# natashabatalha/picaso

Measured on AMD Instinct MI355X. Metric: spectra/sec (1e5 wave x 90 layer reflected), higher is better.
Workload: dtype f64; 1 GPU; BASELINE configs[2]: Toon two-stream reflected light (get_reflected_1d + compress_disco), TTHG_ray, N=2, delta-Eddington, Rayleigh + cloud slab; nwno=100000, nlayer=90, gauss_angles=5, collective=none

## Files before the change

picaso_amd/csrc/api.hip:

```cpp
#include "common.hpp"
#include "planeseal.hpp"

#include <algorithm>
#include <cmath>
#include <cstdlib>

namespace pz {

thread_local char g_err[512] = {0};

int fail(picaso_ctx *ctx, const char *fmt, ...)
{
    char buf[512];
    va_list ap;
    va_start(ap, fmt);
    vsnprintf(buf, sizeof(buf), fmt, ap);
    va_end(ap);
    if (ctx) snprintf(ctx->err, sizeof(ctx->err), "%s", buf);
    snprintf(g_err, sizeof(g_err), "%s", buf);
    return 1;
}

int arena_reset(picaso_ctx *ctx, size_t need)
{
// ... 491 lines not shown
    g.iu0 = 1.0 / v0;
    g.iu0sq = 1.0 / (v0 * v0);
    g.nl0 = NL2E / v0; g.nl1 = NL2E / v1;
    g.nlm = NL2E * (1.0 / v0 + 1.0 / v1);
    g.wq2 = 2.0 * (v0 / (v0 + v1));
    g.q2 = (3.0 * 0.767 * 0.767 * v1 * v1 - 1.0) / 2.0;
    g.wgt = gw;
    g.wgt2 = tw;
    return g;
}

static double refl_dt_small(const double *ubar0, const double *ubar1, int count)
{
    if (getenv("PICASO_AMD_REFL_NO_SMALL_EXP") || !ubar0 || !ubar1 || count < 1) return -1.0;
    double umin = 1.0;
    for (int k = 0; k < count; ++k) {
        const double v0 = fabs(ubar0[k]), v1 = fabs(ubar1[k]);
        if (!(v0 > 0.0) || !(v1 > 0.0)) return -1.0;
        umin = fmin(umin, fmin(v0, v1));
    }
    return 0.34 * umin;
}

struct ReflBatchHost {
    int nspec;
    const double *const *plane[11];
    const double *const *surf_reflect, *const *F0PI;
    double *const *xint, *const *albedo;
    int ngeom;
    const double *cos_theta;
};

static bool reflected_seal_applies(picaso_ctx *ctx, int nlevel, int nwno, long plane_pitch, int numg, int numt,
                                   const double *const one[11], const double *ubar0, const double *ubar1, double cos_theta,
                                   int single_phase, int multi_phase, double frac_c, int toon_coefficients,
                                   const ReflBatchHost *bt, std::vector<unsigned long long> &masks, bool &use_masks)
{
    use_masks = false;
    const int nang = numg * numt, nspec = bt ? bt->nspec : 1, ngeom = bt ? bt->ngeom : 1;
    if (nang != 5) return false;
    for (int s = 0; s < ngeom; ++s) {
        const double ct = bt ? bt->cos_theta[s] : cos_theta;
        const double *u0 = ubar0 + (size_t)s * nang, *u1 = ubar1 + (size_t)s * nang;
        if (ct != 1.0) return false;
        for (int k = 0; k < nang; ++k)
            if (u0[k] != u1[k]) return false;
        if (!picaso_reflected_1d_can_derive(nlevel, plane_pitch, numg, numt, u0, u1, ct, single_phase, multi_phase, frac_c,
                                            toon_coefficients, 0))
            return false;
    }
    long coop_cols = 64L * ctx->ncu;
    if (const char *e = getenv("PICASO_AMD_REFL_COOP_COLS")) coop_cols = atol(e);
    const bool coop = !bt && nwno <= coop_cols && !getenv("PICASO_AMD_REFL_NO_COOP");
    if (!coop) {
        const int group = reflected_angle_group(ctx, nwno, nang, nspec);
        if (group == 1 || (group > 1 && group < nang && ((nang + group - 1) / group) * group <= MAX_ANGLES)) return false;
        if (angle_chunks(nang).size() != 1) return false;
        if ((long)nspec * ((nwno + 255L) / 256) * 4 <= 1024 && !getenv("PICASO_AMD_REFL_NO_BIG")) return false;
    }
    masks.assign(2 * (size_t)nspec, 0ull);
    bool all_valid = true, any_clear = false;
    for (int s = 0; s < nspec; ++s) {
        const double *pl[11];
        for (int j = 0; j < 11; ++j) pl[j] = bt ? bt->plane[j][s] : one[j];
        bool valid = false;
        if (!seal_derivable(ctx->device, pl, nlevel, nwno, plane_pitch, &masks[2 * (size_t)s], &valid)) return false;
        all_valid = all_valid && valid;
        any_clear = any_clear || masks[2 * (size_t)s] || masks[2 * (size_t)s + 1];
    }
    use_masks = !coop && all_valid && any_clear && !getenv("PICASO_AMD_REFL_NO_LAYER_MASK");
    return true;
}

static int reflected_1d_core(picaso_ctx *ctx, int nlevel, int nwno, int ncolper, long plane_pitch, int numg,
                                int numt, const double *dtau, const double *tau, const double *w0,
                                const double *cosb, const double *gcos2, const double *ftau_cld,
                                const double *ftau_ray, const double *dtau_og,
                                const double *tau_og, const double *w0_og, const double *cosb_og,
                                const double *surf_reflect, const double *ubar0,
                                const double *ubar1, double cos_theta, const double *F0PI,
                                int single_phase, int multi_phase, double frac_a, double frac_b,
                                double frac_c, double constant_back, double constant_forward,
                                int get_toa_intensity, int get_lvl_flux, int toon_coefficients,
                                double b_top, double *xint_at_top, double *flux_minus_all,
                                double *flux_plus_all, double *flux_minus_midpt_all,
                                double *flux_plus_midpt_all, const double *gweight,
                                const double *tweight, double *albedo, const ReflBatchHost *bt = nullptr)
{
    if (!ctx) return fail(nullptr, "null context");
    if (nlevel < 2 || nwno < 1 || numg < 1 || numt < 1)
        return fail(ctx, "get_reflected_1d: bad sizes nlevel=%d nwno=%d numg=%d numt=%d", nlevel, nwno, numg, numt);
    if (!dtau || !w0) return fail(ctx, "get_reflected_1d: dtau and w0 are required");
    if (!bt) PZ_NEED(ctx, "get_reflected_1d", surf_reflect, ubar0, ubar1, F0PI, xint_at_top);
    const bool clear_set = !ftau_cld;
    if (clear_set ? (cosb || cosb_og || ftau_ray || gcos2) : (!cosb || !cosb_og || !ftau_ray))
        return fail(ctx, "get_reflected_1d: cosb, cosb_og, ftau_cld, ftau_ray are given together or all left out (gcos2 "
                         "too in the second case)");
    if ((dtau_og == nullptr) != (w0_og == nullptr))
        return fail(ctx, "get_reflected_1d: dtau_og and w0_og are given together or both left out");
    const bool derived = !tau || !tau_og || !gcos2 || !ftau_cld || !dtau_og;
    if (derived && (get_lvl_flux || !get_toa_intensity))
        return fail(ctx, "get_reflected_1d: level fluxes need all eleven planes");
    const int nspec = bt ? bt->nspec : 1;
    const long ncol = (long)nwno * ncolper;
    if (plane_pitch < ncol) return fail(ctx, "get_reflected_1d: plane_pitch %ld < %ld columns", plane_pitch, ncol);
    if (ncolper > 1 && albedo)
        return fail(ctx, "get_reflected_1d: the fused disk sum is a per-wavelength output (ngauss = 1)");
    PZ_TRY(check_phase_options(ctx, single_phase, multi_phase, toon_coefficients));
    PZ_HIP(ctx, hipSetDevice(ctx->device));
    const int nang = numg * numt;
    ReflBatchHost bt_sealed;
    std::vector<const double *> absent;
    std::vector<unsigned long long> lmasks;
    bool use_lmask = false;
    if (!derived && ncolper == 1 && get_toa_intensity && !get_lvl_flux) {
        const double *const pl[11] = {dtau, tau, w0, cosb, gcos2, ftau_cld, ftau_ray, dtau_og, tau_og, w0_og, cosb_og};
        if (reflected_seal_applies(ctx, nlevel, nwno, plane_pitch, numg, numt, pl, ubar0, ubar1, cos_theta, single_phase,
                                   multi_phase, frac_c, toon_coefficients, bt, lmasks, use_lmask)) {
            tau = tau_og = gcos2 = nullptr;
            if (bt) {
                absent.assign((size_t)nspec, nullptr);
                bt_sealed = *bt;
                bt_sealed.plane[1] = bt_sealed.plane[4] = bt_sealed.plane[8] = absent.data();
                bt = &bt_sealed;
            }
            seal_count_hit(ctx->device, use_lmask);
        }
    }
    if (get_lvl_flux) {
        if (!flux_minus_all || !flux_plus_all || !flux_minus_midpt_all || !flux_plus_midpt_all)
            return fail(ctx, "get_reflected_1d: get_lvl_flux=1 needs the four level-flux outputs");
    }
    if (!get_toa_intensity) {
        PZ_HIP(ctx, hipMemsetAsync(xint_at_top, 0, sizeof(double) * (size_t)nang * ncol, ctx->stream));
        if (albedo) PZ_HIP(ctx, hipMemsetAsync(albedo, 0, sizeof(double) * nwno, ctx->stream));
        if (!get_lvl_flux) return 0;
    }
    ReflectedArgs a{};
    a.nlayer = nlevel - 1;
    a.ncol = ncol;
    a.ncolper = ncolper;
    a.pitch = plane_pitch;
    a.nfac = 1;
    a.nwno = nwno;
    a.dtau = dtau; a.tau = tau; a.w0 = w0; a.cosb = cosb; a.gcos2 = gcos2; a.ftau_cld = ftau_cld;
    a.ftau_ray = ftau_ray; a.dtau_og = dtau_og; a.tau_og = tau_og; a.w0_og = w0_og; a.cosb_og = cosb_og;
    a.surf_reflect = surf_reflect; a.F0PI = F0PI; a.cos_theta = cos_theta;
    a.single_phase = single_phase; a.multi_phase = multi_phase; a.toon_coefficients = toon_coefficients;
    a.frac_a = frac_a; a.frac_b = frac_b; a.frac_c = frac_c; a.constant_back = constant_back;
    a.constant_forward = constant_forward; a.b_top = b_top;
    a.use_lmask = use_lmask ? 1 : 0;
    if (use_lmask) { a.lmask[0] = lmasks[0]; a.lmask[1] = lmasks[1]; }
    a.dt_small = refl_dt_small(ubar0, ubar1, (bt ? bt->ngeom : 1) * nang);
    const bool fuse = albedo && gweight && tweight;
    a.albedo = fuse ? albedo : nullptr;
    a.albedo_scale = ((numt == 1) ? 2.0 * 3.14159265358979323846 : 1.0) * 0.5;
    std::vector<ReflBatchItem> items;
    auto upload_batch = [&](int first, int count, bool weights) -> int {
        items.resize((size_t)nspec);
        bool zp = true, ct1 = true;
        for (int s = 0; s < nspec; ++s) {
            ReflBatchItem &it = items[(size_t)s];
            const double *const *P[11];
            for (int j = 0; j < 11; ++j) P[j] = bt->plane[j];
            it.dtau = P[0][s]; it.tau = P[1][s]; it.w0 = P[2][s]; it.cosb = P[3][s]; it.gcos2 = P[4][s];
            it.ftau_cld = P[5][s]; it.ftau_ray = P[6][s]; it.dtau_og = P[7][s]; it.tau_og = P[8][s];
            it.w0_og = P[9][s]; it.cosb_og = P[10][s];
            it.surf_reflect = bt->surf_reflect[s]; it.F0PI = bt->F0PI[s];
            it.xint = bt->xint[s] + (size_t)first * ncol;
            it.albedo = (fuse && weights) ? bt->albedo[s] : nullptr;
            it.cos_theta = bt->cos_theta[bt->ngeom > 1 ? s : 0];
            it.u0_tab = it.u1_tab = nullptr;
            it.lmask[0] = use_lmask ? lmasks[2 * (size_t)s] : 0ull;
            it.lmask[1] = use_lmask ? lmasks[2 * (size_t)s + 1] : 0ull;
            ct1 = ct1 && it.cos_theta == 1.0;
            const double *u0 = ubar0 + (bt->ngeom > 1 ? (size_t)s * nang : 0), *u1 = ubar1 + (bt->ngeom > 1 ? (size_t)s * nang : 0);
            for (int k = 0; k < count; ++k) {
                const int idx = first + k < nang ? first + k : nang - 1;
                it.ang[k] = make_refl_angle(u0[idx], u1[idx], weights ? gweight[idx / numt] : 0.0,
                                            weights ? tweight[idx % numt] : 0.0);
                zp = zp && u0[idx] == u1[idx];
            }
        }
        const void *d = nullptr;
        PZ_TRY(table_upload(ctx, items.data(), sizeof(ReflBatchItem) * items.size(), &d));
        a.batch = (const ReflBatchItem *)d;
        a.nspec = nspec;
        a.batch_zp = zp ? 1 : 0;
        a.cos_theta = ct1 ? 1.0 : bt->cos_theta[0] == 1.0 ? 2.0 : bt->cos_theta[0];
        bool shared = nspec > 1;
        for (int s = 1; s < nspec && shared; ++s)
            for (int j = 0; j < 11; ++j) shared = shared && bt->plane[j][s] == bt->plane[j][0];
        a.batch_interleave = shared ? 1 : 0;
        return 0;
    };
    if (bt) {
        if (get_lvl_flux || !get_toa_intensity)
// ... 1019 lines not shown
```

picaso_amd/csrc/common.hpp:

```cpp
#pragma once
#include <hip/hip_runtime.h>

#include <initializer_list>

#include <unordered_map>

#include <cstdarg>
#include <cstdio>
#include <cstring>
#include <vector>

#include "../../include/picaso_hip.h"

namespace pz { struct PairwisePlan; }

struct picaso_ctx {
    int device = 0;
    hipStream_t stream = nullptr;
    hipEvent_t ev0 = nullptr, ev1 = nullptr;
    hipEvent_t wait_ev = nullptr;
    char err[512] = {0};
    int ncu = 256;
    char *arena = nullptr;
    size_t arena_bytes = 0, arena_used = 0;
// ... 83 lines not shown
constexpr int MAX_CK_GAUSS = 32;

struct ReflectedArgs {
    int nlayer;
    long ncol;
    int ncolper;
    long pitch;
    int nfac;
    int nwno;
    const double *dtau, *tau, *w0, *cosb, *gcos2, *ftau_cld, *ftau_ray, *dtau_og, *tau_og, *w0_og,
        *cosb_og;
    const double *surf_reflect, *F0PI;
    double cos_theta;
    int single_phase, multi_phase, toon_coefficients;
    double frac_a, frac_b, frac_c, constant_back, constant_forward, b_top;
    int na;
    int ny;
    int nvalid;
    int ncg;
    struct Angle {
        double u1, iu0, iu0sq, nl1, q2;
        double u0, nl0, nlm, wq2, wgt, wgt2;
    } ang[MAX_ANGLES];
    const double *u0_tab, *u1_tab;
    double *xint;
    double *albedo;
    double albedo_scale;
    int albedo_first, albedo_last;
    const struct ReflBatchItem *batch;
    int nspec;
    unsigned bps;
    int batch_zp;
    int batch_interleave;
    unsigned long long lmask[2];
    int use_lmask;
    double dt_small;
};
struct ReflBatchItem {
    const double *dtau, *tau, *w0, *cosb, *gcos2, *ftau_cld, *ftau_ray, *dtau_og, *tau_og, *w0_og, *cosb_og;
    const double *surf_reflect, *F0PI;
    double *xint, *albedo;
    double cos_theta;
    const double *u0_tab, *u1_tab;
    ReflectedArgs::Angle ang[MAX_ANGLES];
    unsigned long long lmask[2];
};
int launch_reflected_toa(picaso_ctx *ctx, const ReflectedArgs &a, bool is3d);
bool reflected_coop_ok(const ReflectedArgs &a);
int reflected_coop_pattern(const ReflectedArgs &a);
int launch_reflected_coop(picaso_ctx *ctx, const ReflectedArgs &a);
int launch_weighted_colsum(picaso_ctx *ctx, int nrows, long nwno, int n, const double *wts_host,
                           const double *in, double *out);
int launch_axpby(picaso_ctx *ctx, size_t n, double a, const double *x, double b, const double *y, double *out);


struct ThermalArgs {
    int nlayer;
    long ncol, pitch;
    int nfac, nwno;
    int ncolper;
    const double *wno, *dwno;
    const double *tlevel, *plevel;
    const double *dtau, *w0, *cosb;
    const double *surf_reflect;
    int hard_surface, calc_type;
    int na, ny;
// ... 50 lines not shown
```

picaso_amd/csrc/planeseal.hip:

```cpp
#include "common.hpp"
#include "planeseal.hpp"
#include "planeseal_registry.hpp"

namespace pz {

namespace {

using sealreg::Seal;
static_assert(sealreg::LEVELS_FLAGS == PICASO_SEAL_LEVELS, "planeseal_registry.hpp restates PICASO_SEAL_LEVELS");

sealreg::Registry &registry()
{
    static sealreg::Registry *r = new sealreg::Registry();
    return *r;
}

}

bool seal_derivable(int device, const double *const planes[11], int nlevel, int nwno, long pitch,
                    unsigned long long *layer_mask, bool *mask_valid)
{
    uint64_t m[2];
    const bool ok = registry().derivable(device, planes, nlevel, nwno, pitch, m, mask_valid);
    if (layer_mask) {
        layer_mask[0] = m[0];
        layer_mask[1] = m[1];
    }
    return ok;
}

void seal_count_hit(int device, bool with_layer_mask) { registry().count_hit(device, with_layer_mask); }

void seal_invalidate(int device, const void *p, size_t bytes) { registry().invalidate(device, p, bytes); }

void seal_drop_device(int device) { registry().drop_device(device); }

constexpr int SEAL_BLOCK = 256, SEAL_ROWS = 8;
static_assert(32 % SEAL_ROWS == 0, "the layers of one block lie inside one word of the mask");
constexpr int SEAL_WORDS = 1 + sealreg::MASK_LAYERS / 32;

__global__ __launch_bounds__(SEAL_BLOCK) void k_planes_seal(int nlayer, int nwno, long pitch, const double *dtau,
                                                             const double *tau, const double *gcos2,
                                                             const double *ftau_ray, const double *dtau_og,
                                                             const double *tau_og, const double *w0,
                                                             const double *ftau_cld, const double *w0_og, int *bad_out,
                                                             unsigned *notclear_out)
{
#pragma clang fp contract(off)
    const long col = (long)blockIdx.x * SEAL_BLOCK + threadIdx.x;
    if (col >= nwno) return;
    const int i0 = (int)blockIdx.y * SEAL_ROWS, i1 = (i0 + SEAL_ROWS < nlayer) ? i0 + SEAL_ROWS : nlayer;
    int bad = 0;
    unsigned notclear = 0;
    unsigned lane_cloudy = 0;
    double t = tau[(long)i0 * pitch + col], to = tau_og[(long)i0 * pitch + col];
    if (i0 == 0) {
        if (__double_as_longlong(t) != 0) bad |= PICASO_SEAL_TAU;
        if (__double_as_longlong(to) != 0) bad |= PICASO_SEAL_TAU_OG;
    }
#pragma unroll 4
    for (int i = i0; i < i1; ++i) {
        const long o = (long)i * pitch + col;
        const double tn = tau[o + pitch];
        const double dt = dtau[o], dto = dtau_og[o], fr = ftau_ray[o];
        if (!(tn == t + dt)) bad |= PICASO_SEAL_TAU;
        t = tn;
        if (i + 1 < nlayer) {
            const double ton = tau_og[o + pitch];
            if (!(ton == to + dto)) bad |= PICASO_SEAL_TAU_OG;
            to = ton;
        }
        if (!(gcos2[o] == 0.5 * fr)) bad |= PICASO_SEAL_GCOS2;
        if (notclear_out) {
            const bool cloudy = !(ftau_cld[o] == 0.0) || !(dto == dt) ||
                                __double_as_longlong(fr) != __double_as_longlong(1.0) ||
                                __double_as_longlong(w0_og[o]) != __double_as_longlong(w0[o]);
            if (cloudy) lane_cloudy |= 1u << (i - i0);
        }
    }
#pragma unroll
    for (int b = 0; b < SEAL_ROWS; ++b)
        if (__any((lane_cloudy >> b) & 1u)) notclear |= 1u << ((i0 & 31) + b);
    if (bad) atomicOr(bad_out, bad);
    if (notclear && (threadIdx.x & 63) == 0) atomicOr(notclear_out + (i0 >> 5), notclear);
}

}

using namespace pz;

extern "C" {

int picaso_reflected_planes_seal_dev(picaso_ctx *ctx, int nlevel, int nwno, long plane_pitch, const double *dtau,
                                     const double *tau, const double *w0, const double *cosb, const double *gcos2,
                                     const double *ftau_cld, const double *ftau_ray, const double *dtau_og,
                                     const double *tau_og, const double *w0_og, const double *cosb_og, int *flags_out)
{
    if (!ctx) return fail(nullptr, "null context");
    if (flags_out) *flags_out = 0;
    if (nlevel < 2 || nwno < 1) return fail(ctx, "reflected_planes_seal: bad sizes nlevel=%d nwno=%d", nlevel, nwno);
    if (plane_pitch < nwno) return fail(ctx, "reflected_planes_seal: plane_pitch %ld < %d columns", plane_pitch, nwno);
    PZ_NEED(ctx, "reflected_planes_seal", dtau, tau, w0, cosb, gcos2, ftau_cld, ftau_ray, dtau_og, tau_og, w0_og, cosb_og);
    PZ_HIP(ctx, hipSetDevice(ctx->device));
    void *word = nullptr;
    PZ_TRY(picaso_dev_malloc(ctx, sizeof(int) * SEAL_WORDS, &word));
    int found[SEAL_WORDS] = {0};
    const int nlayer = nlevel - 1;
    const bool with_mask = nlayer <= sealreg::MASK_LAYERS;
    auto run = [&]() -> int {
        PZ_HIP(ctx, hipMemsetAsync(word, 0, sizeof(int) * SEAL_WORDS, ctx->stream));
        const dim3 grid((unsigned)((nwno + SEAL_BLOCK - 1) / SEAL_BLOCK), (unsigned)((nlayer + SEAL_ROWS - 1) / SEAL_ROWS));
        hipLaunchKernelGGL(k_planes_seal, grid, dim3(SEAL_BLOCK), 0, ctx->stream, nlayer, nwno, plane_pitch, dtau, tau,
                           gcos2, ftau_ray, dtau_og, tau_og, w0, ftau_cld, w0_og, (int *)word,
                           with_mask ? (unsigned *)word + 1 : nullptr);
        PZ_HIP(ctx, hipGetLastError());
        PZ_HIP(ctx, hipMemcpyAsync(found, word, sizeof(int) * SEAL_WORDS, hipMemcpyDeviceToHost, ctx->stream));
        PZ_HIP(ctx, hipStreamSynchronize(ctx->stream));
        return 0;
    };
    const int rc = run();
    PZ_TRY(picaso_dev_free(ctx, word));
    if (rc) return rc;
    Seal s{};
    const double *pl[11] = {dtau, tau, w0, cosb, gcos2, ftau_cld, ftau_ray, dtau_og, tau_og, w0_og, cosb_og};
    for (int j = 0; j < 11; ++j) s.plane[j] = pl[j];
    s.nlevel = nlevel;
    s.nwno = nwno;
    s.pitch = plane_pitch;
    s.flags = PICASO_SEAL_LEVELS & ~found[0];
    sealreg::mask_from_device_words(s, with_mask ? (const unsigned *)found + 1 : nullptr);
    registry().record(ctx->device, s);
    if (flags_out) *flags_out = s.flags;
    return 0;
}

int picaso_reflected_planes_unseal(picaso_ctx *ctx, const void *any_plane_ptr)
{
    if (!ctx) return fail(nullptr, "null context");
    seal_invalidate(ctx->device, any_plane_ptr, 1);
    return 0;
}

int picaso_reflected_seal_stat(picaso_ctx *ctx, long *seals, long *hits)
{
    if (!ctx) return fail(nullptr, "null context");
    registry().stat(ctx->device, seals, hits, nullptr);
    return 0;
}

int picaso_reflected_seal_layers(picaso_ctx *ctx, const void *any_plane_ptr, int cap, int *clear_out, int *nlayer_out)
{
    if (!ctx) return fail(nullptr, "null context");
    if (!nlayer_out || cap < 0 || (cap > 0 && !clear_out)) return fail(ctx, "reflected_seal_layers: bad arguments");
// ... 13 lines not shown
```

picaso_amd/csrc/planeseal.hpp:

```cpp
#pragma once
#include <cstddef>

namespace pz {

bool seal_derivable(int device, const double *const planes[11], int nlevel, int nwno, long pitch,
                    unsigned long long *layer_mask = nullptr, bool *mask_valid = nullptr);
void seal_count_hit(int device, bool with_layer_mask = false);
void seal_invalidate(int device, const void *p, size_t bytes);
void seal_drop_device(int device);

}
```

picaso_amd/csrc/planeseal_registry.hpp:

```cpp
#pragma once
#include <atomic>
#include <cstddef>
#include <cstdint>
#include <map>
#include <mutex>
#include <vector>

namespace pz {
namespace sealreg {

constexpr int LEVELS_FLAGS = 7;
constexpr int MASK_LAYERS = 128;

struct Seal {
    const double *plane[11];
    int nlevel, nwno;
    long pitch;
    int flags;
    uint64_t clear[2];
    bool mask_valid;

    size_t extent(int j) const
    {
        const long rows = (j == 1 || j == 8) ? nlevel : nlevel - 1;
        return sizeof(double) * (size_t)((rows - 1) * pitch + nwno);
    }
    bool overlaps(const void *p, size_t bytes) const
    {
        const uintptr_t lo = (uintptr_t)p, hi = lo + bytes;
        for (int j = 0; j < 11; ++j) {
            const uintptr_t q = (uintptr_t)plane[j];
            if (lo < q + extent(j) && q < hi) return true;
        }
        return false;
    }
    bool same_set(const double *const p[11]) const
    {
        for (int j = 0; j < 11; ++j)
            if (plane[j] != p[j]) return false;
        return true;
    }
    bool sealed() const { return (flags & LEVELS_FLAGS) == LEVELS_FLAGS; }
    bool layer_clear(int i) const { return mask_valid && i >= 0 && i < MASK_LAYERS && ((clear[i >> 6] >> (i & 63)) & 1u); }
};

inline void mask_from_device_words(Seal &s, const unsigned *notclear)
{
    const int nlayer = s.nlevel - 1;
    s.clear[0] = s.clear[1] = 0;
    s.mask_valid = notclear != nullptr && nlayer <= MASK_LAYERS;
    if (!s.mask_valid) return;
    for (int i = 0; i < nlayer; ++i)
        if (!((notclear[i >> 5] >> (i & 31)) & 1u)) s.clear[i >> 6] |= (uint64_t)1 << (i & 63);
}

struct DeviceSeals {
    std::vector<Seal> seals;
    long hits = 0;
    long mask_launches = 0;
};

struct Registry {
    std::mutex mu;
    std::map<int, DeviceSeals> dev;
    std::atomic<long> records{0};

    long drop_where(DeviceSeals &d, bool (*pred)(const Seal &, const void *, size_t), const void *p, size_t bytes)
    {
        long n = 0;
        for (size_t k = d.seals.size(); k-- > 0;)
            if (pred(d.seals[k], p, bytes)) {
                d.seals.erase(d.seals.begin() + (long)k);
                ++n;
            }
        records -= n;
        return n;
    }

    void record(int device, const Seal &s)
    {
        std::lock_guard<std::mutex> lock(mu);
        DeviceSeals &d = dev[device];
        drop_where(d, [](const Seal &x, const void *q, size_t) { return x.same_set((const double *const *)q); }, s.plane, 0);
        d.seals.push_back(s);
        ++records;
    }

    bool derivable(int device, const double *const planes[11], int nlevel, int nwno, long pitch, uint64_t *mask,
                   bool *mask_valid)
    {
        if (mask) mask[0] = mask[1] = 0;
        if (mask_valid) *mask_valid = false;
        if (records.load(std::memory_order_relaxed) == 0) return false;
        std::lock_guard<std::mutex> lock(mu);
        auto it = dev.find(device);
        if (it == dev.end()) return false;
        for (const Seal &s : it->second.seals)
            if (s.same_set(planes)) {
                const bool ok = s.nlevel == nlevel && s.nwno == nwno && s.pitch == pitch && s.sealed();
                if (ok && s.mask_valid) {
                    if (mask) {
                        mask[0] = s.clear[0];
                        mask[1] = s.clear[1];
                    }
                    if (mask_valid) *mask_valid = true;
                }
                return ok;
            }
        return false;
    }

    void count_hit(int device, bool with_mask)
    {
        std::lock_guard<std::mutex> lock(mu);
        DeviceSeals &d = dev[device];
        ++d.hits;
        if (with_mask) ++d.mask_launches;
    }

    void invalidate(int device, const void *p, size_t bytes)
    {
        if (!p || !bytes || records.load(std::memory_order_relaxed) == 0) return;
        std::lock_guard<std::mutex> lock(mu);
        auto it = dev.find(device);
        if (it == dev.end()) return;
        drop_where(it->second, [](const Seal &s, const void *q, size_t n) { return s.overlaps(q, n); }, p, bytes);
    }

// ... 41 lines not shown
```

picaso_amd/csrc/toon_reflected.hip:

```cpp
#include "common.hpp"
#include "device_math.hpp"

namespace pz {

#ifndef PZ_REFL_MINWAVES
#define PZ_REFL_MINWAVES 2
#endif
#ifndef PZ_REFL_BLOCK
#define PZ_REFL_BLOCK 256
#endif

constexpr int NSTATE = 7;
enum { S_T = 0, S_XU, S_EO, S_KAPPA, S_ZETA, S_D1, S_D2 };
constexpr int LDS_MIN_ANGLES = 4;

#ifndef PZ_REFL_NLDS
#define PZ_REFL_NLDS 4
#endif

template <int NA, bool LDS>
struct ReflState {
    static constexpr int NL = LDS ? PZ_REFL_NLDS : 0;
    static constexpr int NR = NSTATE - NL;
    double reg[NR > 0 ? NR : 1][NA];
    double *lds;
    double rho, pgam, pEM;
    __device__ __forceinline__ double get(int var, int k) const
    {
        return (var >= NR) ? lds[((var - NR) * NA + k) * PZ_REFL_BLOCK] : reg[var < NR ? var : 0][k];
    }
    __device__ __forceinline__ void set(int var, int k, double v)
    {
        if (var >= NR) lds[((var - NR) * NA + k) * PZ_REFL_BLOCK] = v;
        else reg[var < NR ? var : 0][k] = v;
    }
};

struct LayerIn {
    double dt, tau_n, w0, g, gcos2, fc, fr, dto, tauo, w0o, cbo;
    bool cum_tau;
    bool eo_ok;
    bool same_dt;
    bool nocld;
    bool allf;
    bool af_cloud;
};

enum Body { BODY_GENERAL, BODY_CLOUD, BODY_CLEAR, BODY_CLEAR_TOP, BODY_CLEAR_TOP_SMALL };

template <int NA, bool IS3D, bool ZP, bool FIRST, bool LAST, bool LDS, bool FAST = false, Body KIND = BODY_GENERAL,
          bool XT = false>
__device__ __forceinline__ void reflected_layer(const ReflectedArgs &a, const LayerIn &L,
                                                ReflState<NA, LDS> &S,
                                                const ReflectedArgs::Angle (&g)[NA],
                                                const Exp2Coef &K, double F, double clip, int tc_,
                                                double b_top)
{
#pragma clang fp contract(off)
    constexpr bool NC = KIND >= BODY_CLEAR, AF = KIND != BODY_GENERAL, EOX = KIND >= BODY_CLEAR_TOP;
    constexpr bool SX = KIND == BODY_CLEAR_TOP_SMALL;
    constexpr int SDT = KIND == BODY_CLOUD ? 2 : 1;
    static_assert(!(XT || EOX) || (FAST && ZP), "XT, BODY_CLEAR_TOP*: the zero-phase default-options kernels only");
    const int tc = FAST ? 0 : tc_;
    const int single_phase = FAST ? 3 : a.single_phase;
    const int multi_phase = FAST ? 0 : a.multi_phase;
    const double cos_theta = (FAST && ZP) ? 1.0 : a.cos_theta;
    const double frac_c = FAST ? 2.0 : a.frac_c;
    const double dt = L.dt, w0 = L.w0;
    const double fcg = NC ? 0.0 : L.fc * L.g;
    double g1, g2, lam, lam2;
    if (NC) toon_gammas_nocld(tc, w0, g1, g2, lam, lam2);
    else toon_gammas(tc, w0, fcg, g1, g2, lam, lam2);
    const double E = fmin(lam * dt, clip);
    const double EP = fexp2(E * -NEG_LOG2E, K);
    const double r_ge = frcp(g2 * EP);
    const double ig2 = r_ge * EP, EM = r_ge * g2;
    const double gam = (g1 - lam) * ig2;
    double ps;
    if ((NC || L.nocld) && single_phase == 3)
        ps = L.fr * (0.75 * fma(cos_theta, cos_theta, 1.0));
    else
        ps = p_single<IS3D>(single_phase, L.cbo, L.gcos2, L.fc, L.fr, cos_theta, a.frac_a, a.frac_b,
                            frac_c, a.constant_back, a.constant_forward);
    const double ssa_h = (L.w0o * F * (0.125 / PI)) * ps;
    const double w2pi = w0 * (0.5 / PI);
    const double Fw0h = (0.5 * F) * w0;
    const double gcq = (multi_phase == 0) ? L.gcos2 : 0.0;
    const double c2 = NC ? 0.0 : ((tc == 1) ? 1.5 * fcg : SQ3 * fcg);
    const double A0 = NC ? (g1 + g2) : (g1 + g2) + c2;
    const double A1 = NC ? 0.0 : c2 * (g1 - g2);
    const double c15 = NC ? 0.0 : 1.5 * fcg;
    const double gp = 1.0 + gam;
    const double gmc = NC ? 0.0 : (1.0 - gam) * c15;
    const double w2gp = w2pi * gp, w2gmc = NC ? 0.0 : w2pi * gmc;
    const double w2A0 = w2pi * A0;

    double a1i = 0.0, a2i = 0.0, ia = 0.0, rho_n = gam, sfac = 0.0;
// ... 169 lines not shown
    const double F = a.F0PI[w], rs = a.surf_reflect[w];

    const double *p_dtau = a.dtau + col, *p_tau = a.tau + col, *p_w0 = a.w0 + col,
                 *p_cosb = a.cosb + col, *p_gcos2 = a.gcos2 + col, *p_fc = a.ftau_cld + col,
                 *p_fr = a.ftau_ray + col, *p_dto = a.dtau_og + col, *p_tauo = a.tau_og + col,
                 *p_w0o = a.w0_og + col, *p_cbo = a.cosb_og + col;

    constexpr bool LDS = (NA >= LDS_MIN_ANGLES) && !IS3D && !BIG;
    __shared__ double lds_state[LDS ? (PZ_REFL_NLDS > 0 ? PZ_REFL_NLDS : 1) * NA * PZ_REFL_BLOCK : 1];
    ReflState<NA, LDS> S;
    S.lds = lds_state + threadIdx.x;
    S.rho = S.pgam = S.pEM = 0.0;
    constexpr bool CLEAR = (DRV == 2), LAYERS = (DRV == 4), LEVELS = (DRV == 3) || LAYERS;
    constexpr bool ZDRV = FAST && ZP && !IS3D && (CLEAR || LEVELS);
    constexpr bool TOPRUN = ZDRV && (CLEAR || LAYERS);
    constexpr bool DECKRUN = ZDRV && LAYERS;
    constexpr bool CLEAR_FIRST = TOPRUN, CLEAR_LAST = ZDRV && CLEAR;
    const double dt_small = a.dt_small;
    auto small_dt = [&](double dt) -> bool { return __all(__builtin_fabs(dt) <= dt_small); };
    unsigned long long m0 = 0, m1 = 0;
    if constexpr (LAYERS) {
        m0 = a.lmask[0];
        m1 = a.lmask[1];
    }
    auto layer_clear = [&](int i) -> bool {
        if constexpr (LAYERS) return (((i & 64) ? m1 : m0) >> (i & 63)) & 1ull;
        return false;
    };
    const bool derive_tau = CLEAR || LEVELS || (DRV && a.tau == nullptr);
    const bool derive_tauo = CLEAR || LEVELS || (DRV && a.tau_og == nullptr);
    const bool derive_g2 = CLEAR || LEVELS || (DRV && a.gcos2 == nullptr);
    const bool clear = CLEAR || (!LEVELS && DRV && a.ftau_cld == nullptr);
    const bool alias_og = CLEAR || (!LEVELS && DRV && a.dtau_og == nullptr);
    double tau_i = derive_tau ? 0.0 : p_tau[0];
    double tauo_pred = 0.0;
#pragma unroll
    for (int k = 0; k < NA; ++k) {
        S.set(S_T, k, 1.0);
        S.set(S_KAPPA, k, 0.0);
        S.set(S_ZETA, k, 0.0);
        S.set(S_D1, k, 0.0);
        S.set(S_D2, k, 0.0);
        S.set(S_EO, k, 0.0);
        S.set(S_XU, k, ZDRV ? 1.0 : fexp2(mul_unfused(tau_i, ZP ? g[k].nl1 : g[k].nl0), K));
    }

// ... 131 lines not shown
        prep(L_, lclear_);                                                                               \
        constexpr bool interior_ = !(FIRST_) && !(LAST_);                                                \
         \
                                                              \
        constexpr bool kend_ = !interior_ && (!(FIRST_) || CLEAR_FIRST) && (!(LAST_) || CLEAR_LAST);      \
        constexpr Body kcopy_ = !kend_ ? BODY_GENERAL : (FIRST_) ? BODY_CLEAR_TOP : BODY_CLEAR;          \
        if (kend_ && (CLEAR || lclear_))                                                                 \
            PZ_BODY(FIRST_, LAST_, kcopy_, L_);                                                          \
        else if (FAST && interior_ && L_.nocld && L_.allf)                                               \
            PZ_BODY(FIRST_, LAST_, BODY_CLEAR, L_);                                                      \
        else if (FAST && interior_ && L_.af_cloud)                                                       \
            PZ_BODY(FIRST_, LAST_, BODY_CLOUD, L_);                                                      \
        else                                                                                             \
            PZ_BODY(FIRST_, LAST_, BODY_GENERAL, L_);                                                    \
        if constexpr (CLEAR) __builtin_amdgcn_sched_barrier(0);    \
    } while (0)
#define PZ_RUN_LAYER(KIND_, L_)                                                                          \
    do {                                                                                                 \
        prep(L_, true);                                                                                  \
        PZ_BODY(false, false, KIND_, L_);                                                                \
        __builtin_amdgcn_sched_barrier(0);                                                               \
    } while (0)

    auto load_clear = [&](LayerIn &L, int l) {
        const unsigned o = voff0 + (unsigned)l * pitch8;
        L.dt = ld(a.dtau, o);
        L.w0 = ld(a.w0, o);
    };
    constexpr bool TWO_SETS = (NA <= 2) || (NA == 5 && FAST && ZP);
    LayerIn A, B;
    load(A, 0);
    if (n == 1) {
        PZ_LAYER(true, true, A, 0);
    } else if constexpr (TWO_SETS) {
        load(B, 1);
        PZ_LAYER(true, false, A, 0);
        int i = 1;
        if constexpr (TOPRUN) {
            int r = n;
            if constexpr (LAYERS) {
                r = (~m0) ? __builtin_ctzll(~m0) : 64 + ((~m1) ? __builtin_ctzll(~m1) : 64);
                r = r < n ? r : n;
            }
            if (r >= 1) {
                if (i + 2 < r) {
                    double dt_a = ld(a.dtau, voff0 + (unsigned)(i + 1) * pitch8);
                    bool go = small_dt(B.dt) && small_dt(dt_a);
                    while (go) {
                        A.dt = dt_a;
                        A.w0 = ld(a.w0, voff0 + (unsigned)(i + 1) * pitch8);
                        PZ_RUN_LAYER(BODY_CLEAR_TOP_SMALL, B);
                        load_clear(B, i + 2);
                        dt_a = ld(a.dtau, voff0 + (unsigned)(i + 3 < n ? i + 3 : n - 1) * pitch8);
                        PZ_RUN_LAYER(BODY_CLEAR_TOP_SMALL, A);
                        i += 2;
                        go = i + 2 < r && small_dt(B.dt) && small_dt(dt_a);
                    }
                }
                for (; i + 2 < r; i += 2) {
                    load_clear(A, i + 1);
                    PZ_RUN_LAYER(BODY_CLEAR_TOP, B);
                    load_clear(B, i + 2);
                    PZ_RUN_LAYER(BODY_CLEAR_TOP, A);
                }
#pragma unroll
                for (int k = 0; k < NA; ++k) S.set(S_EO, k, S.get(S_XU, k));
            }
        }
        for (; i + 2 <= n - 1; i += 2) {
            if constexpr (DECKRUN) {
                const unsigned long long w = i < 64 ? (m0 >> i) | (i ? m1 << (64 - i) : 0ull) : m1 >> (i - 64);
                int e = i + ((~w) ? __builtin_ctzll(~w) : 64);
                e = e < n - 1 ? e : n - 1;
                if (i + 2 < e) {
                    for (; i + 2 < e; i += 2) {
                        load_clear(A, i + 1);
                        PZ_RUN_LAYER(BODY_CLEAR, B);
                        load_clear(B, i + 2);
                        PZ_RUN_LAYER(BODY_CLEAR, A);
                    }
                    if (!(i + 2 <= n - 1)) break;
                }
            }
            load(A, i + 1, true);
            PZ_LAYER(false, false, B, i);
            load(B, i + 2, true);
            PZ_LAYER(false, false, A, i + 1);
        }
        if (i == n - 1) {
            PZ_LAYER(false, true, B, i);
        } else {
            load(A, i + 1, true);
            PZ_LAYER(false, false, B, i);
            PZ_LAYER(false, true, A, i + 1);
        }
    } else {
        load(B, 1);
        PZ_LAYER(true, false, A, 0);
        for (int i = 1; i < n - 1; ++i) {
            A = B;
            load(B, i + 1);
            PZ_LAYER(false, false, A, i);
        }
        A = B;
        PZ_LAYER(false, true, A, n - 1);
    }
#undef PZ_LAYER
#undef PZ_RUN_LAYER
#undef PZ_BODY

    double alb = (!IS3D && a.albedo && !a.albedo_first) ? a.albedo[w] : 0.0;
    double xout[NA];
    {
#pragma clang fp contract(off)
        const double em2 = S.pEM * S.pEM;
        const double bden = 1.0 / fma(-(em2 * (S.pgam - rs)), S.rho, fma(-rs, S.pgam, 1.0));
#pragma unroll
        for (int k = 0; k < NA; ++k) {
            const double b_surface = ((rs * (ZP ? g[k].u1 : g[k].u0)) * F) * S.get(S_XU, k);
            const double pos = (S.pEM * fma(rs, S.get(S_D2, k), b_surface - S.get(S_D1, k))) * bden;
            xout[k] = fma(S.get(S_ZETA, k), pos, S.get(S_KAPPA, k));
        }
    }
#pragma unroll
    for (int k = 0; k < NA; ++k) {
        const double x = xout[k];
        if (IS3D) a.xint[(long)fac * a.nwno + w] = x;
        else if (NA == 1 || (int)by * NA + k < a.nvalid) a.xint[(long)(by * NA + k) * a.ncol + col] = x;
        alb = disk_accumulate(alb, x, g[k].wgt, g[k].wgt2);
    }
    if (!IS3D && a.albedo) {
// ... 28 lines not shown
template <int NA, bool IS3D, bool ZP, bool FAST = false, bool BIG = false, int DRV = 0>
__global__ __launch_bounds__(PZ_REFL_BLOCK, (BIG ? 1 : PZ_REFL_MINWAVES)) void k_reflected_toa_batch(const ReflectedArgs a)
{
    unsigned spec, bx, by = 0;
    const unsigned ny = a.ny > 1 ? (unsigned)a.ny : 1u;
    if (!IS3D && a.batch_interleave) {
        unsigned rep;
        xcd_decode(blockIdx.x, ny * (unsigned)a.nspec, (unsigned)a.ncg, rep, bx);
        spec = rep / ny;
        by = rep - spec * ny;
    } else {
        spec = blockIdx.x / a.bps;
        bx = blockIdx.x - spec * a.bps;
        if (!IS3D && ny > 1) xcd_decode(bx, ny, (unsigned)a.ncg, by, bx);
    }
    typedef const __attribute__((address_space(4))) ReflBatchItem *ItemPtr;
    const auto &it = *((ItemPtr)(unsigned long)a.batch + spec);
    ReflectedArgs b = a;
    b.dtau = it.dtau; b.tau = it.tau; b.w0 = it.w0; b.cosb = it.cosb; b.gcos2 = it.gcos2; b.ftau_cld = it.ftau_cld;
    b.ftau_ray = it.ftau_ray; b.dtau_og = it.dtau_og; b.tau_og = it.tau_og; b.w0_og = it.w0_og; b.cosb_og = it.cosb_og;
    b.surf_reflect = it.surf_reflect; b.F0PI = it.F0PI; b.xint = it.xint; b.albedo = it.albedo;
    b.cos_theta = it.cos_theta;
    b.u0_tab = it.u0_tab; b.u1_tab = it.u1_tab;
    if constexpr (DRV == 4) { b.lmask[0] = it.lmask[0]; b.lmask[1] = it.lmask[1]; }
    reflected_toa_body<NA, IS3D, ZP, FAST, BIG, DRV>(b, bx, by, it.ang);
}

static bool fast_options(const ReflectedArgs &a, bool zp)
{
    if (getenv("PICASO_AMD_REFL_GENERIC")) return false;
    if ((double)a.pitch * (a.nlayer + 1) * 8.0 >= 4294967296.0) return false;
    return a.toon_coefficients == 0 && a.single_phase == 3 && a.multi_phase == 0 && (!zp || a.cos_theta == 1.0) &&
           a.frac_c == 2.0;
}

template <int NA, bool IS3D, bool ZP, bool FAST = false, bool BIG = false, int DRV = 0>
static void launch_kernel(picaso_ctx *ctx, const dim3 grid, const ReflectedArgs &a)
{
    if (a.batch)
        hipLaunchKernelGGL((k_reflected_toa_batch<NA, IS3D, ZP, FAST, BIG, DRV>), grid, dim3(PZ_REFL_BLOCK), 0, ctx->stream, a);
    else
        hipLaunchKernelGGL((k_reflected_toa<NA, IS3D, ZP, FAST, BIG, DRV>), grid, dim3(PZ_REFL_BLOCK), 0, ctx->stream, a);
}

template <int NA>
static int launch1d(picaso_ctx *ctx, const ReflectedArgs &a_in)
{
// ... 80 lines not shown
```

Baseline: 5903 spectra/s.

## Add cloud-deck layer runs and small-argument exp path to reflected kernel

Extends the plane-seal kernel to record a per-layer cloud-deck mask and a flag that all w0 lie in [0,1], then uses these in the reflected TOA kernel. Runs of deck layers take a dedicated cloud loop that loads only the needed planes and fixes the per-layer flags at compile time. Clear top layers with a provably small exponent argument use a cheaper fexp2_small. The u0_tab/u1_tab pointers now share a union with the new cmask field, which adds state and a risk of aliasing mistakes if the tables are ever needed together with the masks.

New measurement: 5969 spectra/s, median of 6. 1.1% higher.

```diff
diff --git a/picaso_amd/csrc/api.hip b/picaso_amd/csrc/api.hip
--- a/picaso_amd/csrc/api.hip
+++ b/picaso_amd/csrc/api.hip
@@ -537,6 +537,13 @@
     return 0.34 * umin;
 }
 
+static bool refl_ep_small(const double *ubar0, const double *ubar1, int count)
+{
+    const double dts = refl_dt_small(ubar0, ubar1, count);
+    if (!(dts >= 0.0)) return false;
+    return dts * 1.7320508075688772935 * 1.4426950408889634074 * (1.0 + 0x1p-40) <= 0.5;
+}
+
 struct ReflBatchHost {
     int nspec;
     const double *const *plane[11];
@@ -549,9 +556,11 @@
 static bool reflected_seal_applies(picaso_ctx *ctx, int nlevel, int nwno, long plane_pitch, int numg, int numt,
                                    const double *const one[11], const double *ubar0, const double *ubar1, double cos_theta,
                                    int single_phase, int multi_phase, double frac_c, int toon_coefficients,
-                                   const ReflBatchHost *bt, std::vector<unsigned long long> &masks, bool &use_masks)
+                                   const ReflBatchHost *bt, std::vector<unsigned long long> &masks, bool &use_masks,
+                                   std::vector<unsigned long long> &cmasks, bool &w0_unit)
 {
     use_masks = false;
+    w0_unit = false;
     const int nang = numg * numt, nspec = bt ? bt->nspec : 1, ngeom = bt ? bt->ngeom : 1;
     if (nang != 5) return false;
     for (int s = 0; s < ngeom; ++s) {
@@ -574,16 +583,21 @@
         if ((long)nspec * ((nwno + 255L) / 256) * 4 <= 1024 && !getenv("PICASO_AMD_REFL_NO_BIG")) return false;
     }
     masks.assign(2 * (size_t)nspec, 0ull);
-    bool all_valid = true, any_clear = false;
+    cmasks.assign(2 * (size_t)nspec, 0ull);
+    bool all_valid = true, any_clear = false, all_unit = true;
     for (int s = 0; s < nspec; ++s) {
         const double *pl[11];
         for (int j = 0; j < 11; ++j) pl[j] = bt ? bt->plane[j][s] : one[j];
-        bool valid = false;
-        if (!seal_derivable(ctx->device, pl, nlevel, nwno, plane_pitch, &masks[2 * (size_t)s], &valid)) return false;
+        bool valid = false, unit = false;
+        if (!seal_derivable(ctx->device, pl, nlevel, nwno, plane_pitch, &masks[2 * (size_t)s], &valid,
+                            &cmasks[2 * (size_t)s], &unit))
+            return false;
         all_valid = all_valid && valid;
+        all_unit = all_unit && unit;
         any_clear = any_clear || masks[2 * (size_t)s] || masks[2 * (size_t)s + 1];
     }
     use_masks = !coop && all_valid && any_clear && !getenv("PICASO_AMD_REFL_NO_LAYER_MASK");
+    w0_unit = use_masks && all_unit;
     return true;
 }
 
@@ -627,11 +641,12 @@
     ReflBatchHost bt_sealed;
     std::vector<const double *> absent;
     std::vector<unsigned long long> lmasks;
-    bool use_lmask = false;
+    std::vector<unsigned long long> cmasks;
+    bool use_lmask = false, w0_unit = false;
     if (!derived && ncolper == 1 && get_toa_intensity && !get_lvl_flux) {
         const double *const pl[11] = {dtau, tau, w0, cosb, gcos2, ftau_cld, ftau_ray, dtau_og, tau_og, w0_og, cosb_og};
         if (reflected_seal_applies(ctx, nlevel, nwno, plane_pitch, numg, numt, pl, ubar0, ubar1, cos_theta, single_phase,
-                                   multi_phase, frac_c, toon_coefficients, bt, lmasks, use_lmask)) {
+                                   multi_phase, frac_c, toon_coefficients, bt, lmasks, use_lmask, cmasks, w0_unit)) {
             tau = tau_og = gcos2 = nullptr;
             if (bt) {
                 absent.assign((size_t)nspec, nullptr);
@@ -667,6 +682,9 @@
     a.use_lmask = use_lmask ? 1 : 0;
     if (use_lmask) { a.lmask[0] = lmasks[0]; a.lmask[1] = lmasks[1]; }
     a.dt_small = refl_dt_small(ubar0, ubar1, (bt ? bt->ngeom : 1) * nang);
+    const bool cloud_runs = use_lmask && !getenv("PICASO_AMD_REFL_NO_CLOUD_RUNS");
+    if (cloud_runs) { a.cmask[0] = cmasks[0]; a.cmask[1] = cmasks[1]; }
+    a.ep_small = (cloud_runs && w0_unit && refl_ep_small(ubar0, ubar1, (bt ? bt->ngeom : 1) * nang)) ? 1 : 0;
     const bool fuse = albedo && gweight && tweight;
     a.albedo = fuse ? albedo : nullptr;
     a.albedo_scale = ((numt == 1) ? 2.0 * 3.14159265358979323846 : 1.0) * 0.5;
@@ -688,6 +706,8 @@
             it.u0_tab = it.u1_tab = nullptr;
             it.lmask[0] = use_lmask ? lmasks[2 * (size_t)s] : 0ull;
             it.lmask[1] = use_lmask ? lmasks[2 * (size_t)s + 1] : 0ull;
+            it.cmask[0] = cloud_runs ? cmasks[2 * (size_t)s] : 0ull;
+            it.cmask[1] = cloud_runs ? cmasks[2 * (size_t)s + 1] : 0ull;
             ct1 = ct1 && it.cos_theta == 1.0;
             const double *u0 = ubar0 + (bt->ngeom > 1 ? (size_t)s * nang : 0), *u1 = ubar1 + (bt->ngeom > 1 ? (size_t)s * nang : 0);
             for (int k = 0; k < count; ++k) {
diff --git a/picaso_amd/csrc/common.hpp b/picaso_amd/csrc/common.hpp
--- a/picaso_amd/csrc/common.hpp
+++ b/picaso_amd/csrc/common.hpp
@@ -129,7 +129,10 @@
         double u1, iu0, iu0sq, nl1, q2;
         double u0, nl0, nlm, wq2, wgt, wgt2;
     } ang[MAX_ANGLES];
-    const double *u0_tab, *u1_tab;
+    union {
+        struct { const double *u0_tab, *u1_tab; };
+        unsigned long long cmask[2];
+    };
     double *xint;
     double *albedo;
     double albedo_scale;
@@ -141,6 +144,7 @@
     int batch_interleave;
     unsigned long long lmask[2];
     int use_lmask;
+    int ep_small;
     double dt_small;
 };
 struct ReflBatchItem {
@@ -148,7 +152,10 @@
     const double *surf_reflect, *F0PI;
     double *xint, *albedo;
     double cos_theta;
-    const double *u0_tab, *u1_tab;
+    union {
+        struct { const double *u0_tab, *u1_tab; };
+        unsigned long long cmask[2];
+    };
     ReflectedArgs::Angle ang[MAX_ANGLES];
     unsigned long long lmask[2];
 };
diff --git a/picaso_amd/csrc/planeseal.hip b/picaso_amd/csrc/planeseal.hip
--- a/picaso_amd/csrc/planeseal.hip
+++ b/picaso_amd/csrc/planeseal.hip
@@ -18,13 +18,17 @@
 }
 
 bool seal_derivable(int device, const double *const planes[11], int nlevel, int nwno, long pitch,
-                    unsigned long long *layer_mask, bool *mask_valid)
+                    unsigned long long *layer_mask, bool *mask_valid, unsigned long long *deck_mask, bool *w0_unit)
 {
-    uint64_t m[2];
-    const bool ok = registry().derivable(device, planes, nlevel, nwno, pitch, m, mask_valid);
+    uint64_t m[2], c[2];
+    const bool ok = registry().derivable(device, planes, nlevel, nwno, pitch, m, mask_valid, c, w0_unit);
     if (layer_mask) {
         layer_mask[0] = m[0];
         layer_mask[1] = m[1];
+    }
+    if (deck_mask) {
+        deck_mask[0] = c[0];
+        deck_mask[1] = c[1];
     }
     return ok;
 }
@@ -37,7 +41,8 @@
 
 constexpr int SEAL_BLOCK = 256, SEAL_ROWS = 8;
 static_assert(32 % SEAL_ROWS == 0, "the layers of one block lie inside one word of the mask");
-constexpr int SEAL_WORDS = 1 + sealreg::MASK_LAYERS / 32;
+constexpr int SEAL_MASK_WORDS = sealreg::MASK_LAYERS / 32;
+constexpr int SEAL_WORDS = 1 + 2 * SEAL_MASK_WORDS + 1;
 
 __global__ __launch_bounds__(SEAL_BLOCK) void k_planes_seal(int nlayer, int nwno, long pitch, const double *dtau,
                                                              const double *tau, const double *gcos2,
@@ -53,6 +58,8 @@
     int bad = 0;
     unsigned notclear = 0;
     unsigned lane_cloudy = 0;
+    unsigned notdeck = 0, lane_notdeck = 0;
+    bool w0_out = false;
     double t = tau[(long)i0 * pitch + col], to = tau_og[(long)i0 * pitch + col];
     if (i0 == 0) {
         if (__double_as_longlong(t) != 0) bad |= PICASO_SEAL_TAU;
@@ -72,17 +79,29 @@
         }
         if (!(gcos2[o] == 0.5 * fr)) bad |= PICASO_SEAL_GCOS2;
         if (notclear_out) {
-            const bool cloudy = !(ftau_cld[o] == 0.0) || !(dto == dt) ||
+            const double fc = ftau_cld[o], w = w0[o];
+            const bool cloudy = !(fc == 0.0) || !(dto == dt) ||
                                 __double_as_longlong(fr) != __double_as_longlong(1.0) ||
-                                __double_as_longlong(w0_og[o]) != __double_as_longlong(w0[o]);
+                                __double_as_longlong(w0_og[o]) != __double_as_longlong(w);
             if (cloudy) lane_cloudy |= 1u << (i - i0);
+            if (fc == 0.0 || dto == dt) lane_notdeck |= 1u << (i - i0);
+            if (!(w >= 0.0 && w <= 1.0)) w0_out = true;
         }
     }
 #pragma unroll
     for (int b = 0; b < SEAL_ROWS; ++b)
         if (__any((lane_cloudy >> b) & 1u)) notclear |= 1u << ((i0 & 31) + b);
+#pragma unroll
+    for (int b = 0; b < SEAL_ROWS; ++b)
+        if (__any((lane_notdeck >> b) & 1u)) notdeck |= 1u << ((i0 & 31) + b);
+    const bool any_w0_out = __any(w0_out);
     if (bad) atomicOr(bad_out, bad);
     if (notclear && (threadIdx.x & 63) == 0) atomicOr(notclear_out + (i0 >> 5), notclear);
+    if (notclear_out && (threadIdx.x & 63) == 0) {
+        unsigned *deck_word = notclear_out + SEAL_MASK_WORDS + (i0 >> 5), *w0_word = notclear_out + 2 * SEAL_MASK_WORDS;
+        if (notdeck & ~__hip_atomic_load(deck_word, __ATOMIC_RELAXED, __HIP_MEMORY_SCOPE_AGENT)) atomicOr(deck_word, notdeck);
+        if (any_w0_out && !__hip_atomic_load(w0_word, __ATOMIC_RELAXED, __HIP_MEMORY_SCOPE_AGENT)) atomicOr(w0_word, 1u);
+    }
 }
 
 }
@@ -128,7 +147,9 @@
     s.nwno = nwno;
     s.pitch = plane_pitch;
     s.flags = PICASO_SEAL_LEVELS & ~found[0];
-    sealreg::mask_from_device_words(s, with_mask ? (const unsigned *)found + 1 : nullptr);
+    sealreg::mask_from_device_words(s, with_mask ? (const unsigned *)found + 1 : nullptr,
+                                    with_mask ? (const unsigned *)found + 1 + SEAL_MASK_WORDS : nullptr,
+                                    with_mask && found[1 + 2 * SEAL_MASK_WORDS] == 0);
     registry().record(ctx->device, s);
     if (flags_out) *flags_out = s.flags;
     return 0;
diff --git a/picaso_amd/csrc/planeseal.hpp b/picaso_amd/csrc/planeseal.hpp
--- a/picaso_amd/csrc/planeseal.hpp
+++ b/picaso_amd/csrc/planeseal.hpp
@@ -4,7 +4,8 @@
 namespace pz {
 
 bool seal_derivable(int device, const double *const planes[11], int nlevel, int nwno, long pitch,
-                    unsigned long long *layer_mask = nullptr, bool *mask_valid = nullptr);
+                    unsigned long long *layer_mask = nullptr, bool *mask_valid = nullptr,
+                    unsigned long long *deck_mask = nullptr, bool *w0_unit = nullptr);
 void seal_count_hit(int device, bool with_layer_mask = false);
 void seal_invalidate(int device, const void *p, size_t bytes);
 void seal_drop_device(int device);
diff --git a/picaso_amd/csrc/planeseal_registry.hpp b/picaso_amd/csrc/planeseal_registry.hpp
--- a/picaso_amd/csrc/planeseal_registry.hpp
+++ b/picaso_amd/csrc/planeseal_registry.hpp
@@ -19,6 +19,8 @@
     int flags;
     uint64_t clear[2];
     bool mask_valid;
+    uint64_t deck[2];
+    bool w0_unit;
 
     size_t extent(int j) const
     {
@@ -44,14 +46,21 @@
     bool layer_clear(int i) const { return mask_valid && i >= 0 && i < MASK_LAYERS && ((clear[i >> 6] >> (i & 63)) & 1u); }
 };
 
-inline void mask_from_device_words(Seal &s, const unsigned *notclear)
+inline void mask_from_device_words(Seal &s, const unsigned *notclear, const unsigned *notdeck = nullptr,
+                                   bool w0_unit = false)
 {
     const int nlayer = s.nlevel - 1;
     s.clear[0] = s.clear[1] = 0;
+    s.deck[0] = s.deck[1] = 0;
+    s.w0_unit = false;
     s.mask_valid = notclear != nullptr && nlayer <= MASK_LAYERS;
     if (!s.mask_valid) return;
-    for (int i = 0; i < nlayer; ++i)
-        if (!((notclear[i >> 5] >> (i & 31)) & 1u)) s.clear[i >> 6] |= (uint64_t)1 << (i & 63);
+    s.w0_unit = w0_unit;
+    for (int i = 0; i < nlayer; ++i) {
+        const bool clear = !((notclear[i >> 5] >> (i & 31)) & 1u);
+        if (clear) s.clear[i >> 6] |= (uint64_t)1 << (i & 63);
+        if (!clear && notdeck && !((notdeck[i >> 5] >> (i & 31)) & 1u)) s.deck[i >> 6] |= (uint64_t)1 << (i & 63);
+    }
 }
 
 struct DeviceSeals {
@@ -87,10 +96,12 @@
     }
 
     bool derivable(int device, const double *const planes[11], int nlevel, int nwno, long pitch, uint64_t *mask,
-                   bool *mask_valid)
+                   bool *mask_valid, uint64_t *deck = nullptr, bool *w0_unit = nullptr)
     {
         if (mask) mask[0] = mask[1] = 0;
         if (mask_valid) *mask_valid = false;
+        if (deck) deck[0] = deck[1] = 0;
+        if (w0_unit) *w0_unit = false;
         if (records.load(std::memory_order_relaxed) == 0) return false;
         std::lock_guard<std::mutex> lock(mu);
         auto it = dev.find(device);
@@ -104,6 +115,11 @@
                         mask[1] = s.clear[1];
                     }
                     if (mask_valid) *mask_valid = true;
+                    if (deck) {
+                        deck[0] = s.deck[0];
+                        deck[1] = s.deck[1];
+                    }
+                    if (w0_unit) *w0_unit = s.w0_unit;
                 }
                 return ok;
             }
diff --git a/picaso_amd/csrc/toon_reflected.hip b/picaso_amd/csrc/toon_reflected.hip
--- a/picaso_amd/csrc/toon_reflected.hip
+++ b/picaso_amd/csrc/toon_reflected.hip
@@ -46,7 +46,7 @@
     bool af_cloud;
 };
 
-enum Body { BODY_GENERAL, BODY_CLOUD, BODY_CLEAR, BODY_CLEAR_TOP, BODY_CLEAR_TOP_SMALL };
+enum Body { BODY_GENERAL, BODY_CLOUD, BODY_CLEAR, BODY_CLEAR_TOP, BODY_CLEAR_TOP_SMALL, BODY_CLEAR_TOP_SMALL_EP };
 
 template <int NA, bool IS3D, bool ZP, bool FIRST, bool LAST, bool LDS, bool FAST = false, Body KIND = BODY_GENERAL,
           bool XT = false>
@@ -58,7 +58,7 @@
 {
 #pragma clang fp contract(off)
     constexpr bool NC = KIND >= BODY_CLEAR, AF = KIND != BODY_GENERAL, EOX = KIND >= BODY_CLEAR_TOP;
-    constexpr bool SX = KIND == BODY_CLEAR_TOP_SMALL;
+    constexpr bool SX = KIND >= BODY_CLEAR_TOP_SMALL, SEP = KIND == BODY_CLEAR_TOP_SMALL_EP;
     constexpr int SDT = KIND == BODY_CLOUD ? 2 : 1;
     static_assert(!(XT || EOX) || (FAST && ZP), "XT, BODY_CLEAR_TOP*: the zero-phase default-options kernels only");
     const int tc = FAST ? 0 : tc_;
@@ -72,7 +72,7 @@
     if (NC) toon_gammas_nocld(tc, w0, g1, g2, lam, lam2);
     else toon_gammas(tc, w0, fcg, g1, g2, lam, lam2);
     const double E = fmin(lam * dt, clip);
-    const double EP = fexp2(E * -NEG_LOG2E, K);
+    const double EP = SEP ? fexp2_small(E * -NEG_LOG2E, K) : fexp2(E * -NEG_LOG2E, K);
     const double r_ge = frcp(g2 * EP);
     const double ig2 = r_ge * EP, EM = r_ge * g2;
     const double gam = (g1 - lam) * ig2;
@@ -288,6 +288,11 @@
     if constexpr (LAYERS) {
         m0 = a.lmask[0];
         m1 = a.lmask[1];
+    }
+    unsigned long long c0 = 0, c1 = 0;
+    if constexpr (LAYERS) {
+        c0 = a.cmask[0];
+        c1 = a.cmask[1];
     }
     auto layer_clear = [&](int i) -> bool {
         if constexpr (LAYERS) return (((i & 64) ? m1 : m0) >> (i & 63)) & 1ull;
@@ -465,6 +470,29 @@
         __builtin_amdgcn_sched_barrier(0);                                                               \
     } while (0)
 
+#define PZ_CLOUD_LAYER(L_)                                                                               \
+    do {                                                                                                 \
+        L_.gcos2 = 0.5 * L_.fr;                                                                          \
+        L_.tau_n = tau_i + L_.dt;                                                                        \
+        L_.tauo = tauo_pred;                                                                             \
+        L_.cum_tau = L_.eo_ok = L_.af_cloud = true;                                                      \
+        L_.same_dt = L_.nocld = L_.allf = false;                                                         \
+        tau_i = L_.tau_n;                                                                                \
+        tauo_pred = L_.tauo + L_.dto;                                                                    \
+        PZ_BODY(false, false, BODY_CLOUD, L_);                                                           \
+        __builtin_amdgcn_sched_barrier(0);                                                               \
+    } while (0)
+    auto load_cloud = [&](LayerIn &L, int l) {
+        const unsigned o = voff0 + (unsigned)l * pitch8;
+        L.dt = ld(a.dtau, o);
+        L.w0 = ld(a.w0, o);
+        L.g = ld(a.cosb, o);
+        L.fc = ld(a.ftau_cld, o);
+        L.fr = ld(a.ftau_ray, o);
+        L.cbo = ld(a.cosb_og, o);
+        L.dto = ld(a.dtau_og, o);
+        L.w0o = ld(a.w0_og, o);
+    };
     auto load_clear = [&](LayerIn &L, int l) {
         const unsigned o = voff0 + (unsigned)l * pitch8;
         L.dt = ld(a.dtau, o);
@@ -489,16 +517,22 @@
                 if (i + 2 < r) {
                     double dt_a = ld(a.dtau, voff0 + (unsigned)(i + 1) * pitch8);
                     bool go = small_dt(B.dt) && small_dt(dt_a);
-                    while (go) {
-                        A.dt = dt_a;
-                        A.w0 = ld(a.w0, voff0 + (unsigned)(i + 1) * pitch8);
-                        PZ_RUN_LAYER(BODY_CLEAR_TOP_SMALL, B);
-                        load_clear(B, i + 2);
-                        dt_a = ld(a.dtau, voff0 + (unsigned)(i + 3 < n ? i + 3 : n - 1) * pitch8);
-                        PZ_RUN_LAYER(BODY_CLEAR_TOP_SMALL, A);
-                        i += 2;
-                        go = i + 2 < r && small_dt(B.dt) && small_dt(dt_a);
+#define PZ_SMALL_LOOP(KIND_)                                                                             \
+                    while (go) {                                                                         \
+                        A.dt = dt_a;                                                                     \
+                        A.w0 = ld(a.w0, voff0 + (unsigned)(i + 1) * pitch8);                             \
+                        PZ_RUN_LAYER(KIND_, B);                                                          \
+                        load_clear(B, i + 2);                                                            \
+                        dt_a = ld(a.dtau, voff0 + (unsigned)(i + 3 < n ? i + 3 : n - 1) * pitch8);       \
+                        PZ_RUN_LAYER(KIND_, A);                                                          \
+                        i += 2;                                                                          \
+                        go = i + 2 < r && small_dt(B.dt) && small_dt(dt_a);                              \
                     }
+                    if constexpr (LAYERS) {
+                        if (a.ep_small) PZ_SMALL_LOOP(BODY_CLEAR_TOP_SMALL_EP)
+                    }
+                    PZ_SMALL_LOOP(BODY_CLEAR_TOP_SMALL)
+#undef PZ_SMALL_LOOP
                 }
                 for (; i + 2 < r; i += 2) {
                     load_clear(A, i + 1);
@@ -512,6 +546,18 @@
         }
         for (; i + 2 <= n - 1; i += 2) {
             if constexpr (DECKRUN) {
+                const unsigned long long wc = i < 64 ? (c0 >> i) | (i ? c1 << (64 - i) : 0ull) : c1 >> (i - 64);
+                int ec = i + ((~wc) ? __builtin_ctzll(~wc) : 64);
+                ec = ec < n - 1 ? ec : n - 1;
+                if (i + 2 <= ec) {
+                    for (; i + 2 <= ec; i += 2) {
+                        load_cloud(A, i + 1);
+                        PZ_CLOUD_LAYER(B);
+                        load_cloud(B, i + 2);
+                        PZ_CLOUD_LAYER(A);
+                    }
+                    if (!(i + 2 <= n - 1)) break;
+                }
                 const unsigned long long w = i < 64 ? (m0 >> i) | (i ? m1 << (64 - i) : 0ull) : m1 >> (i - 64);
                 int e = i + ((~w) ? __builtin_ctzll(~w) : 64);
                 e = e < n - 1 ? e : n - 1;
@@ -550,6 +596,7 @@
     }
 #undef PZ_LAYER
 #undef PZ_RUN_LAYER
+#undef PZ_CLOUD_LAYER
 #undef PZ_BODY
 
     double alb = (!IS3D && a.albedo && !a.albedo_first) ? a.albedo[w] : 0.0;
@@ -624,7 +671,10 @@
     b.surf_reflect = it.surf_reflect; b.F0PI = it.F0PI; b.xint = it.xint; b.albedo = it.albedo;
     b.cos_theta = it.cos_theta;
     b.u0_tab = it.u0_tab; b.u1_tab = it.u1_tab;
-    if constexpr (DRV == 4) { b.lmask[0] = it.lmask[0]; b.lmask[1] = it.lmask[1]; }
+    if constexpr (DRV == 4) {
+        b.lmask[0] = it.lmask[0]; b.lmask[1] = it.lmask[1];
+        b.cmask[0] = it.cmask[0]; b.cmask[1] = it.cmask[1];
+    }
     reflected_toa_body<NA, IS3D, ZP, FAST, BIG, DRV>(b, bx, by, it.ang);
 }
 
```
